# ouyangjiahong/representation-disentanglement

Measured on AMD Instinct MI355X. Metric: MR slices/sec (train step, recon+adv+latent losses), higher is better.
Workload: dtype f32

## Files before the change

representation-disentanglement_amd/csrc/mrdis_common.h:

```cpp
#pragma once
#include <hip/hip_runtime.h>
#include <stdint.h>
#include "../../include/mrdis.h"
#include "mrdis_device.h"
#include "mrdis_launchers.h"

#define MRDIS_CHECK_LAUNCH()                                     \
    do {                                                         \
        hipError_t e_ = hipGetLastError();                       \
        if (e_ != hipSuccess) return MRDIS_ELAUNCH;              \
    } while (0)

#define MRDIS_OPTIONS(X) \
    X(WINO, "wino", "MRDIS_WINO", 0, 1)  \
    X(NT_MB, "nt_mb", "MRDIS_NT_MB", 0, 128)  \
    X(WINO_PIPE, "wino_pipe", "MRDIS_WINO_PIPE", 0, 1)  \
    X(WINO_U, "wino_u", "MRDIS_WINO_U", 0, 1)  \
    X(WINO4, "wino4", "MRDIS_WINO4", 0, 1)  \
    X(WINO4R, "wino4r", "MRDIS_WINO4R", 0, 1)  \
    X(BCONV4, "bconv4", "MRDIS_BCONV4", 0, 1)  \
    X(SPLIT6, "split6", "MRDIS_SPLIT6", 0, 1)  \
    X(NO16, "debug_no16", "MRDIS_DEBUG_NO16", 1, 0) \
    X(NOTHIN, "debug_nothin", "MRDIS_DEBUG_NOTHIN", 1, 0) \
    X(NOC4, "debug_noc4", "MRDIS_DEBUG_NOC4", 1, 0) \
    X(NODMA, "debug_nodma", "MRDIS_DEBUG_NODMA", 1, 0) \
    X(NO16_3D, "debug_no16_3d", "MRDIS_DEBUG_NO16_3D", 1, 0) \
    X(BILGEN, "debug_bilgen", "MRDIS_DEBUG_BILGEN", 1, 0) \
    X(NOW16, "debug_now16", "MRDIS_DEBUG_NOW16", 1, 0) \
    X(NOPACK, "debug_nopack", "MRDIS_DEBUG_NOPACK", 1, 0)  \
    X(MODE, "debug_mode", "MRDIS_DEBUG_MODE", 0, -1) \
    X(BN, "debug_bn", "MRDIS_DEBUG_BN", 0, -1) \
    X(KC, "debug_kc", "MRDIS_DEBUG_KC", 0, -1) \
    X(BM, "debug_bm", "MRDIS_DEBUG_BM", 0, -1) \
    X(C4_TW, "debug_c4_tw", "MRDIS_DEBUG_C4_TW", 0, -1) \
    X(WGSPLIT, "debug_wgsplit", "MRDIS_DEBUG_WGSPLIT", 0, -1) \
    X(BN3, "debug_bn3", "MRDIS_DEBUG_BN3", 0, -1) \
    X(KC3, "debug_kc3", "MRDIS_DEBUG_KC3", 0, -1) \
    X(C4_GRID, "c4_grid", "MRDIS_C4_GRID", 0, 0)  \
    X(C4_BLOCKS, "debug_c4_blocks", "MRDIS_DEBUG_C4_BLOCKS", 0, -1)  \
    X(ZS_GRID, "zsearch_grid", "MRDIS_ZSEARCH_GRID", 0, 0)  \
    X(VOLGEN, "debug_volgen", "MRDIS_DEBUG_VOLGEN", 1, 0)
#define MRDIS_X_OPT_ID(id, name, env, is_flag, dflt) MRDIS_OPT_##id,
enum { MRDIS_OPTIONS(MRDIS_X_OPT_ID) MRDIS_OPT_COUNT };
long long mrdis_opt(int id);
void mrdis_opt_note(int id, long long value);

#define MRDIS_COUNTERS(X) \
    X(WINO, "wino") X(WINO_SPADE, "wino_spade") X(WINO2, "wino2") X(WINO2_SPADE, "wino2_spade") X(WINO4, "wino4") X(WINO4_SPADE, "wino4_spade") X(WINO4N, "wino4n") \
    X(WINO4R, "wino4r") X(WINO_WGRAD, "wino_wgrad") X(WINO_WGRAD2, "wino_wgrad2") X(WINO4_WGRAD, "wino4_wgrad") X(BCONV3, "bconv3") X(BCONV3_SPADE, "bconv3_spade") \
    X(BCONV4, "bconv4") X(BCONV4_SPADE, "bconv4_spade") X(SPLIT6_C4, "split6_c4") X(SPLIT6_C16, "split6_c16") X(SPLIT6_WGRAD16, "split6_wgrad16") X(SPLIT6_CO4, "split6_co4") \
    X(SPLIT6_C3D, "split6_c3d") X(SPLIT6_W3D, "split6_w3d") X(SPLIT6_TAP, "split6_tap") X(ZSEARCH, "zsearch") \
    X(CONV2SRC, "conv2src") X(ANA_ACT, "ana_act")  \
    X(KL, "kl") X(AVGPOOL, "avgpool")  \
    X(CHATT, "chatt") X(SYMDIFF, "symdiff") X(RGATE, "rgate")  \
    X(DIRECT3D, "direct3d") X(C3D16, "c3d16") X(WGRAD3D, "wgrad3d") X(WGRAD3D16, "wgrad3d16") X(WINO_WGRAD3D, "wino_wgrad3d")  \
    X(VOLGATHER, "volgather")  \
    X(FGCOUNT, "fgcount") X(PATCHORIGIN, "patchorigin") X(PATCHGATHER, "patchgather")  \
    X(PATCHWARP, "patchwarp")  \
    X(LOSS3D, "loss3d") X(SEGCOUNTS, "segcounts")  \
    X(SEGACCUM, "segaccum") X(SEGLABELS, "seglabels")  \
    X(TILEACCUM, "tileaccum") X(TILELABELS, "tilelabels")  \
    X(SYNTHACCUM, "synthaccum") X(SYNTHFINISH, "synthfinish")  \
    X(SEG2DLABELS, "seg2dlabels") X(SEG2DFINISH, "seg2dfinish")  \
    X(FUSE, "fuse")  \
    X(REGSURF, "regsurf") X(EDT, "edt") X(SURFHIST, "surfhist")  \
    X(CCLABEL, "cclabel") X(CCCLEAN, "ccclean")  \
// ... 39 lines not shown
```

representation-disentanglement_amd/csrc/mrdis_conv.hip:

```cpp
#include "mrdis_common.h"
#include "mrdis_tapconv.h"
#include "mrdis_s6conv.h"
#include "mrdis_wino4.h"
#include <stdlib.h>
#include <type_traits>

__device__ float g_mrdis_zero_page[64];
#define TC_TAB_INTS 320

template <int KC, int BN, int MODE, int BM, int SK = 1>
__device__ __forceinline__ void tapconv_body(const TapConvParams& p, const int bx, const int gx) {
    constexpr int S = KC + 1;
    constexpr int WAVES_N = (BN == 32) ? 1 : 2;
    constexpr int WAVES_M = 4 / WAVES_N;
    constexpr int MSUB = (BM / 32) / WAVES_M;
    constexpr int NSUB = (BN / 32) / WAVES_N;
    constexpr int KCW = KC / SK;
    static_assert(SK == 1 || (SK == 2 && BN == 32 && BM == 128 && MODE == 1 && KC >= 8), "split-K form: 64 positions x 32 couts, two waves per 32 x 32 block");
    extern __shared__ __attribute__((aligned(16))) float smem[];
    int* tab_in = reinterpret_cast<int*>(smem);
    int* tab_out = tab_in + BM;
    int* tap_xoff = tab_in + 2 * BM;
    int* tap_widx = tab_in + 2 * BM + 16;
    float* ws = smem + (2 * BM + 64);
// ... 2268 lines not shown
    WgradPlan pl;
    if (plan_wgrad(pl, N, H, W, Ci, Ci, Co, kh, kw, stride, pad)) return 0;
    size_t need = wgrad_need(pl);
    { const size_t nb = mrdis_bwgrad_workspace(N, H, W, Ci, Co, kh, kw, stride, pad); if (nb > need) need = nb; }
    if (kh == 3 && kw == 3 && stride == 1 && pad == 1) {
        const size_t nw = mrdis_wino_wgrad_workspace(N, H, W, Ci, Co);
        if (nw > need) need = nw;
        const size_t n16 = mrdis_wgrad16_workspace(N, H, W, Ci, Co);
        if (n16 > need) need = n16;
        const size_t n4 = mrdis_wgrad_c4_workspace(N, H, W, Ci, Co);
        if (n4 > need) need = n4;
        const size_t n4b = mrdis_wgrad_co4b_workspace(N, H, W, Ci, Co);
        if (n4b > need) need = n4b;
    }
    { const size_t n2 = mrdis_wgrad_s2_workspace(N, H, W, Ci, Co, kh, kw, stride, pad); if (n2 > need) need = n2; }
    if (kh == 1 && kw == 1 && stride == 1 && pad == 0) { const size_t n1 = mrdis_pw_wgrad_workspace((long long)N * H * W, Ci, Co, 1); if (n1 > need) need = n1; }
    return need;
}

template <int J>
static int launch_wgrad_t(const WgradPlan& pl, hipStream_t s) {
    if (pl.dma) {
        if (!mrdis_lds_optin((const void*)wgrad_dma_kernel<J>, 96 * 1024)) return MRDIS_ELAUNCH;
        const bool x_ok = (pl.p.ldx % 4 == 0) && (((uintptr_t)pl.p.x & 15) == 0);
        const bool dy_ok = (pl.p.lddy % 4 == 0) && (((uintptr_t)pl.p.dy & 15) == 0);
        if (x_ok && dy_ok) {
            MRDIS_LAUNCH((wgrad_dma_kernel<J>), dim3(pl.p.splits * pl.p.base), dim3(256), pl.lds_dma, s, pl.p, pl.XR);
            MRDIS_CHECK_LAUNCH();
            return MRDIS_OK;
        }
// ... 40 lines not shown
    if (kh == 3 && kw == 3 && stride == 1 && pad == 1 && Ci == 4) {
        rc = mrdis_run_wgrad_c4(x, ldx, dy, lddy, dw_tck, dbias, workspace, workspace_bytes, N, H, W, Ci, Co, accumulate_bias, 0, (hipStream_t)stream);
        if (rc != MRDIS_EUNSUPPORTED) return rc;
    }
    if (kh == 3 && kw == 3 && stride == 1 && pad == 1 && Co <= 16) {
        rc = mrdis_run_wgrad16(x, ldx, dy, lddy, dw_tck, dbias, workspace, workspace_bytes, N, H, W, Ci, Co, accumulate_bias, (hipStream_t)stream);
        if (rc != MRDIS_EUNSUPPORTED) return rc;
    }
    if (kh == 1 && kw == 1 && stride == 1 && pad == 0) {
        rc = mrdis_run_pw_wgrad(x, ldx, dy, lddy, dw_tck, dbias, workspace, workspace_bytes, (long long)N * H * W, Ci, Co, accumulate_bias, 0, (hipStream_t)stream);
        if (rc != MRDIS_EUNSUPPORTED) return rc;
    }
    if (stride == 2 && Ci <= 7) {
        rc = mrdis_run_wgrad_s2(x, ldx, dy, lddy, dw_tck, dbias, workspace, workspace_bytes, N, H, W, Ci, Co, kh, kw, stride, pad, accumulate_bias,
                                (hipStream_t)stream);
        if (rc != MRDIS_EUNSUPPORTED) return rc;
    }
    if (wino_wgrad_wanted(N, H, W, Ci, Co, kh, kw, stride, pad)) {
        rc = mrdis_run_wino_wgrad(x, ldx, dy, lddy, dw_tck, dbias, workspace, workspace_bytes, N, H, W, Ci, Co, accumulate_bias, (hipStream_t)stream);
        if (rc != MRDIS_EUNSUPPORTED) return rc;
    }
    hipStream_t s = (hipStream_t)stream;
    WgradParams& p = pl.p;
    p.x = x; p.dy = dy; p.ldx = ldx; p.lddy = lddy;
    p.slab = reinterpret_cast<float*>(workspace);
    float* part = p.slab + pl.slab_floats;
    p.bias_slab = dbias ? part + pl.part_floats : nullptr;
    p.vec_x = (Ci % 4 == 0) && (ldx % 4 == 0) && (((uintptr_t)x & 15) == 0) && (p.CW % 4 == 0);
    p.vec_dy = (Co % 4 == 0) && (lddy % 4 == 0) && (((uintptr_t)dy & 15) == 0);
    const bool x_al = (ldx % 4 == 0) && (((uintptr_t)x & 15) == 0), dy_al = (lddy % 4 == 0) && (((uintptr_t)dy & 15) == 0);
// ... 486 lines not shown
```

representation-disentanglement_amd/csrc/mrdis_launchers.h:

```cpp
#pragma once
#include <hip/hip_runtime.h>
#include <stddef.h>

int mrdis_run_wino(const float* x, int ldx, const float* w, const float* bias, float* y, int ldy,
                   int N, int H, int W, int Ci, int Co, int flip, int lrelu, hipStream_t s);
int mrdis_run_wino3d(const float* x, int ldx, const float* w, const float* bias, const float* res, int ldres, float* y, int ldy,
                     int N, int D, int H, int W, int Ci, int Co, int flip, hipStream_t s);
size_t mrdis_wino_wgrad_workspace(int N, int H, int W, int Ci, int Co);
int mrdis_run_wino_wgrad(const float* x, int ldx, const float* dy, int lddy, float* dw_tck, float* dbias, void* workspace,
                         size_t workspace_bytes, int N, int H, int W, int Ci, int Co, int accumulate_bias, hipStream_t s);
size_t mrdis_wino_wgrad3d_workspace(int N, int D, int H, int W, int Ci, int Co);
int mrdis_run_wino_wgrad3d(const float* x, int ldx, const float* dy, int lddy, float* dw_tck, float* dbias, void* workspace,
                           size_t workspace_bytes, int N, int D, int H, int W, int Ci, int Co, hipStream_t s);

int mrdis_run_wino2(const float* x, int ldx, const float* w, const float* bias, float* y, int ldy,
                    int N, int H, int W, int Ci, int Co, int flip, int lrelu, hipStream_t s, const float* u_img);
int mrdis_run_wino2_spade(const float* x, int ldx, const float* w, const float* bias, const float* z, int ldz, const float* mean, const float* rstd,
                          float* mix, int ldmix, float* gamma, int ldg, int N, int H, int W, int Ci, int C, hipStream_t s, const float* u_img);

int mrdis_run_wino4(const float* x, int ldx, const float* bias, float* y, int ldy, int N, int H, int W, int Ci, int Co, int lrelu,
                    hipStream_t s, const float* u_img);
int mrdis_run_wino4n(const float* x, int ldx, const float* bias, float* y, int ldy, int N, int H, int W, int Ci, int Co, int lrelu,
                     hipStream_t s, const float* u_img);
int mrdis_run_wino4_spade(const float* x, int ldx, const float* bias, const float* z, int ldz, const float* mean, const float* rstd,
                          float* mix, int ldmix, float* gamma, int ldg, int N, int H, int W, int Ci, int C, hipStream_t s, const float* u_img);
// ... 48 lines not shown
```

representation-disentanglement_amd/csrc/mrdis_wino.h:

```cpp
#pragma once
#include "mrdis_common.h"

struct WinoWgradParams {
    const float* x; const float* dy; float* slab; float* bias_slab;
    int N, H, W, Ci, ldx, Co, lddy;
    int nby, nbx, nblocks;
    int nCiB, nCoB, splits;
    int D, kd;
};

int mrdis_launch_wino_wgrad2(const WinoWgradParams& p, hipStream_t s);

int mrdis_launch_wino4_wgrad(WinoWgradParams& p, int max_splits, hipStream_t s);
```

representation-disentanglement_amd/csrc/mrdis_wino.hip:

```cpp
#include "mrdis_common.h"
#include "mrdis_wino.h"
#include <stdlib.h>

struct WinoParams {
    const float* in; const float* w; const float* bias; float* out;
    const float* res; int ldres;
    int D;
    int N, H, W, Cin, ldin, Cout, ldout;
    int flip, lrelu, nt_out;
    int TBH, TBW;
    int nby, nbx, coTiles;
};

template <int CG, int TG, bool D3 = false>
__global__ __launch_bounds__(64 * CG * TG, (CG * TG == 8) ? 1 : 2) void wino_conv_kernel(const WinoParams p) {
    constexpr int KC = 8, NT = 64 * CG * TG;
    constexpr int RWP = 24;
    constexpr int BN = 32 * CG, T = 16 * TG;
    constexpr int TS = T + 16, US = BN + 16;
    constexpr int XR = NT == 512 ? 2 : 3;
    constexpr int UR = (KC * BN) / NT;
    extern __shared__ __attribute__((aligned(16))) float smem[];
    float* U = smem;
    float* V = U + 16 * KC * US;
// ... 443 lines not shown
        __syncthreads();
        float s_ = 0.f;
#pragma unroll
        for (int z = 0; z < ZR; ++z) s_ += bsum[z];
        float* red = smem;
        red[tid] = (tid < TB * COB || ZR > 1) ? s_ : 0.f;
        __syncthreads();
        if (tid < COB) {
            float t = 0.f;
            for (int k = tid; k < NT; k += COB) t += red[k];
            p.bias_slab[(long long)split * p.Co + co0 + tid] = t;
        }
    }
}

__global__ void wino_sum_slabs_kernel(const float* __restrict__ slab, float* __restrict__ dw, long long n, int nslab,
                                      const float* __restrict__ bslab, float* __restrict__ dbias, int Co, int accumulate_bias) {
    __shared__ float red[16][65];
    const long long i = (long long)blockIdx.x * 64 + threadIdx.x;
    const int SL = blockDim.y, y = threadIdx.y;
    float s_ = 0.f;
    if (i < n) {
        const float* src = slab + i + (long long)y * n;
        const long long step = (long long)SL * n;
        int k = y;
        for (; k + 3 * SL < nslab; k += 4 * SL, src += 4 * step) { const float a = src[0], b = src[step], c = src[2 * step], d = src[3 * step]; s_ += a; s_ += b; s_ += c; s_ += d; }
        for (; k < nslab; k += SL, src += step) s_ += *src;
    } else if (dbias != nullptr && i < n + Co) {
        const int co = (int)(i - n);
        for (int k = y; k < nslab; k += SL) s_ += bslab[(long long)k * Co + co];
    }
    red[y][threadIdx.x] = s_;
    __syncthreads();
    if (y == 0) {
        float t = 0.f;
        for (int k = 0; k < SL; ++k) t += red[k][threadIdx.x];
        if (i < n) dw[i] = t;
        else if (dbias != nullptr && i < n + Co) { const int co = (int)(i - n); dbias[co] = accumulate_bias ? dbias[co] + t : t; }
    }
}

struct WinoWgradPlan { WinoWgradParams p; int wci, wco; size_t lds; bool ok; };

static void plan_wino_wgrad(WinoWgradPlan& pl, int N, int H, int W, int Ci, int Co) {
    pl.ok = false;
    int wci, wco;
    if (Ci % 64 == 0 && Co % 64 == 0) { wci = 4; wco = 2; }
    else if (Ci % 64 == 0 && Co % 32 == 0) { wci = 4; wco = 1; }
    else if (Ci % 32 == 0 && Co % 64 == 0) { wci = 2; wco = 2; }
    else return;
    WinoWgradParams& p = pl.p;
    p = WinoWgradParams{};
// ... 2 lines not shown
    const long long nb = (long long)N * p.nby * p.nbx;
    if (nb > 0x7fffffffLL) return;
    p.nblocks = (int)nb;
    const int CIB = 16 * wci, COB = 32 * wco;
    p.nCiB = Ci / CIB; p.nCoB = Co / COB;
    const int target = (wci * wco == 8) ? 256 : 512;
    int splits = target / (p.nCiB * p.nCoB);
    if (splits < 1) splits = 1;
    if (splits > p.nblocks) splits = p.nblocks;
    p.splits = splits;
    pl.wci = wci; pl.wco = wco;
    pl.lds = sizeof(float) * ((size_t)16 * 8 * (CIB + 16) + (size_t)16 * 8 * (COB + 16) + (size_t)60 * (CIB + 4));
    pl.ok = true;
}

size_t mrdis_wino_wgrad_workspace(int N, int H, int W, int Ci, int Co) {
    WinoWgradPlan pl;
    plan_wino_wgrad(pl, N, H, W, Ci, Co);
    if (!pl.ok) return 0;
    return sizeof(float) * ((size_t)pl.p.splits * 9 * Ci * Co + (size_t)pl.p.splits * Co) + 256;
}

int mrdis_run_wino_wgrad(const float* x, int ldx, const float* dy, int lddy, float* dw_tck, float* dbias, void* workspace,
                         size_t workspace_bytes, int N, int H, int W, int Ci, int Co, int accumulate_bias, hipStream_t s) {
    WinoWgradPlan pl;
    plan_wino_wgrad(pl, N, H, W, Ci, Co);
    if (!pl.ok || ldx % 4 != 0 || (((uintptr_t)x) & 15) != 0) return MRDIS_EUNSUPPORTED;
    if (workspace_bytes < mrdis_wino_wgrad_workspace(N, H, W, Ci, Co) - 256) return MRDIS_EUNSUPPORTED;
    WinoWgradParams& p = pl.p;
    p.x = x; p.dy = dy; p.ldx = ldx; p.lddy = lddy;
    p.slab = reinterpret_cast<float*>(workspace);
    p.bias_slab = dbias ? p.slab + (size_t)p.splits * 9 * Ci * Co : nullptr;
    int rc2 = MRDIS_EUNSUPPORTED;
    {
        const int rc4 = mrdis_launch_wino4_wgrad(p, p.splits, s);
        if (rc4 == MRDIS_OK) rc2 = MRDIS_OK;
        else if (rc4 != MRDIS_EUNSUPPORTED) return rc4;
    }
    const int nblk = p.splits * p.nCiB * p.nCoB;
    if (rc2 != MRDIS_OK && pl.wci == 4 && pl.wco == 2 && mrdis_opt(MRDIS_OPT_WINO_PIPE)) {
        rc2 = mrdis_launch_wino_wgrad2(p, s);
        if (rc2 != MRDIS_OK && rc2 != MRDIS_EUNSUPPORTED) return rc2;
    }
#define WW_LAUNCH(a, b_, nt, kb) { if (!mrdis_lds_optin((const void*)wino_wgrad_kernel<a, b_>, kb * 1024)) return MRDIS_ELAUNCH; \
                                   mrdis_count(MRDIS_CNT_WINO_WGRAD); MRDIS_LAUNCH((wino_wgrad_kernel<a, b_>), dim3(nblk), dim3(nt), pl.lds, s, p); }
    if (rc2 == MRDIS_OK) {}
    else if (pl.wci == 4 && pl.wco == 2) WW_LAUNCH(4, 2, 512, 120)
    else if (pl.wci == 4) WW_LAUNCH(4, 1, 256, 80)
    else WW_LAUNCH(2, 2, 256, 80)
#undef WW_LAUNCH
    MRDIS_CHECK_LAUNCH();
    const long long n = 9LL * Ci * Co;
    int SL = 1;
    while (SL < 16 && SL * 4 <= p.splits) SL <<= 1;
    MRDIS_LAUNCH(wino_sum_slabs_kernel, dim3(mrdis_cdiv(n + (dbias ? Co : 0), 64)), dim3(64, SL), 0, s, p.slab, dw_tck, n, p.splits,
                       p.bias_slab, dbias, Co, accumulate_bias);
    MRDIS_CHECK_LAUNCH();
    return MRDIS_OK;
}

size_t mrdis_wino_wgrad3d_workspace(int N, int D, int H, int W, int Ci, int Co) { return mrdis_wino_wgrad_workspace(N * D, H, W, Ci, Co); }

int mrdis_run_wino_wgrad3d(const float* x, int ldx, const float* dy, int lddy, float* dw_tck, float* dbias, void* workspace,
                           size_t workspace_bytes, int N, int D, int H, int W, int Ci, int Co, hipStream_t s) {
    WinoWgradPlan pl;
    plan_wino_wgrad(pl, N * D, H, W, Ci, Co);
    if (!pl.ok || ldx % 4 != 0 || (((uintptr_t)x) & 15) != 0) return MRDIS_EUNSUPPORTED;
    if (workspace_bytes + 256 < mrdis_wino_wgrad3d_workspace(N, D, H, W, Ci, Co)) return MRDIS_EUNSUPPORTED;
    WinoWgradParams& p = pl.p;
    p.x = x; p.dy = dy; p.ldx = ldx; p.lddy = lddy; p.D = D;
    p.slab = reinterpret_cast<float*>(workspace);
// ... 3 lines not shown
                             : (const void*)wino_wgrad_kernel<2, 2, true>, w42 ? 120 * 1024 : 80 * 1024)) return MRDIS_ELAUNCH;
    const int nblk = p.splits * p.nCiB * p.nCoB;
    const long long n = 9LL * Ci * Co;
    int SL = 1;
    while (SL < 16 && SL * 4 <= p.splits) SL <<= 1;
    for (int kd = 0; kd < 3; ++kd) {
        p.kd = kd;
        p.bias_slab = (dbias && kd == 1) ? bias_slab : nullptr;
        mrdis_count(MRDIS_CNT_WINO_WGRAD3D);
        if (w42) MRDIS_LAUNCH((wino_wgrad_kernel<4, 2, true>), dim3(nblk), dim3(512), pl.lds, s, p);
        else if (pl.wci == 4) MRDIS_LAUNCH((wino_wgrad_kernel<4, 1, true>), dim3(nblk), dim3(256), pl.lds, s, p);
        else MRDIS_LAUNCH((wino_wgrad_kernel<2, 2, true>), dim3(nblk), dim3(256), pl.lds, s, p);
        MRDIS_CHECK_LAUNCH();
        float* db = p.bias_slab ? dbias : nullptr;
        MRDIS_LAUNCH(wino_sum_slabs_kernel, dim3(mrdis_cdiv(n + (db ? Co : 0), 64)), dim3(64, SL), 0, s, p.slab, dw_tck + kd * n, n, p.splits,
                           p.bias_slab, db, Co, 0);
        MRDIS_CHECK_LAUNCH();
    }
    return MRDIS_OK;
}
```

representation-disentanglement_amd/csrc/mrdis_wino4w.hip:

```cpp
#include "mrdis_wino.h"

namespace {
constexpr int W_NT = 512;
constexpr int W_VPP = 256, W_VBUF = 18 * W_VPP;
constexpr int W_ZPP = 512, W_ZBUF = 18 * W_ZPP;
constexpr int W_PIX = 32, W_RAW = 128 * W_PIX;
constexpr int W_NXI = 4;
constexpr size_t W4W_LDS = sizeof(float) * (2 * W_VBUF + 2 * W_ZBUF + 3 * W_RAW);
template <int V_> struct WIC { static constexpr int value = V_; };
__device__ __forceinline__ f32x2 ww_ld2(const float* p) { return *(const volatile __attribute__((address_space(3))) f32x2*)p; }
__device__ __forceinline__ void ww_st2(float* p, f32x2 v) { *(volatile __attribute__((address_space(3))) f32x2*)p = v; }
constexpr unsigned WW_OOB = 0xfffffff0u;
}

struct Wino4WgradParams {
    const float* x; const float* dy; float* slab; float* bias_slab;
    int N, H, W, Ci, ldx, Co, lddy;
    int ngy, ngx, ngroups;
    int nCiB, nCoB, splits;
    int prio;
    int s_n, s_gy, s_gx;
    unsigned long long* dbg; int dbg_cap;
};

__global__ __launch_bounds__(512, 2) void wino4_wgrad_kernel(const Wino4WgradParams p) {
    extern __shared__ __attribute__((aligned(16))) float smem[];
    float* const Vb = smem;
    float* const Zb = smem + 2 * W_VBUF;
    float* const Rb = Zb + 2 * W_ZBUF;

    const int tid = threadIdx.x, lane = tid & 63, l16 = lane & 15, kq = lane >> 4;
    const int wave = __builtin_amdgcn_readfirstlane(tid >> 6);
    int b_ = mrdis_xcd_remap((int)blockIdx.x, (int)gridDim.x);
    const int cob = b_ % p.nCoB; b_ /= p.nCoB;
    const int cib = b_ % p.nCiB;
    const int split = b_ / p.nCiB;
    const int ci0 = 32 * cib, co0 = 64 * cob;
    const int wi = wave & 1, wo = wave >> 1;
    const int a_off = kq * 64 + ((2 * (16 * wi + l16) + 32 * kq) & 63);
// ... 4 lines not shown
    const int p0_ = (4 * ty) * 10 + 4 * tx;
    const int v_src0 = p0_ * W_PIX + 4 * ((vc >> 2) ^ (p0_ & 4)) + (vc & 3);
    const int v_src1 = p0_ * W_PIX + 4 * ((vc >> 2) ^ (p0_ & 4) ^ 4) + (vc & 3);
    const int v_dst = t_ * 64 + ((2 * vc + 32 * t_) & 63);
    const int zc = 16 * (wave & 3) + l16;
    const int z_dst = t_ * 128 + ((2 * zc + 32 * t_) & 127);

    struct Cur { int n, gy, gx; };
    auto advance = [&](Cur& c) {
        c.gx += p.s_gx; if (c.gx >= p.ngx) { c.gx -= p.ngx; ++c.gy; }
        c.gy += p.s_gy; if (c.gy >= p.ngy) { c.gy -= p.ngy; ++c.n; }
        c.n += p.s_n;
    };
    Cur xcur, dcur;
    { int t = split; xcur.gx = t % p.ngx; t /= p.ngx; xcur.gy = t % p.ngy; xcur.n = t / p.ngy; dcur = xcur; }
    const __amdgpu_buffer_rsrc_t rs_x = mrdis_buffer_rsrc(p.x, mrdis_nhwc_bytes(p.N, p.H, p.W, p.ldx, p.Ci, 4));
    const __amdgpu_buffer_rsrc_t rs_dy = mrdis_buffer_rsrc(p.dy, mrdis_nhwc_bytes(p.N, p.H, p.W, p.lddy, p.Co, 4));

    float sc[62];
#pragma unroll
    for (int k = 0; k < 62; ++k) sc[k] = 0.f;
#define WW_D(ii, j) sc[5 * ((j) & 1) + (ii)]
#define WW_R(a, j) sc[10 + 6 * (a) + (j)]
#define WW_VO(k) sc[28 + (k)]
#define WW_DY(S, e) sc[16 * (S) + (e)]
#define WW_T(i, j) sc[32 + 4 * (i) + (j)]
#define WW_ZO(k) sc[56 + (k)]
    float bsum = 0.f;
    if ((p.prio == 1 && wave >= 4) || (p.prio == 2 && wave < 4)) __builtin_amdgcn_s_setprio(1);

    unsigned x_rel[W_NXI]; int x_yx[W_NXI];
#pragma unroll
    for (int j = 0; j < W_NXI; ++j) {
        const int slot = 8 * ((wave & 3) + 4 * j) + (lane >> 3), q = (lane & 7) ^ (slot & 4), ry = slot / 10, rx = slot - ry * 10;
        x_yx[j] = slot < 100 ? ((ry << 8) | rx) : -1;
        x_rel[j] = 4u * (unsigned)((ry * p.W + rx) * p.ldx + ci0 + 4 * q);
    }
    const unsigned lds_raw = (unsigned)(size_t)(__attribute__((address_space(3))) void*)Rb;
    auto dma_x = [&](int buf, int j) {
        const int h = 8 * xcur.gy - 1 + (x_yx[j] >> 8), w_ = 8 * xcur.gx - 1 + (x_yx[j] & 255);
        const bool ok = x_yx[j] >= 0 && xcur.n < p.N && (unsigned)h < (unsigned)p.H && (unsigned)w_ < (unsigned)p.W;
        const unsigned gb = 4u * (unsigned)(((xcur.n * p.H + 8 * xcur.gy - 1) * p.W + 8 * xcur.gx - 1) * p.ldx);
        const unsigned vo = ok ? gb + x_rel[j] : WW_OOB;
        const unsigned m0v = __builtin_amdgcn_readfirstlane(lds_raw + 4u * (unsigned)(buf * W_RAW) + 1024u * (unsigned)((wave & 3) + 4 * j));
        mrdis_buffer_lds_dma16(m0v, vo, rs_x);
        if (j == W_NXI - 1) advance(xcur);
    };
    auto v_read = [&](const float* Rr, int j, auto RH_) {
#pragma unroll
        for (int ii = 0; ii < 5; ++ii) { const int d_ = (decltype(RH_)::value + ii) * 10 + j; WW_D(ii, j) = Rr[((d_ & 4) ? v_src1 : v_src0) + d_ * W_PIX]; }
    };
    auto v_col = [&](int j, auto RH_) {
        const float e0 = WW_D(0, j), e1 = WW_D(1, j), e2 = WW_D(2, j), e3 = WW_D(3, j), e4 = WW_D(4, j);
        if constexpr (decltype(RH_)::value == 0) {
            const float a = fmaf(-4.f, e2, e4), b = fmaf(-4.f, e1, e3);
            WW_R(0, j) = fmaf(4.f, e0, fmaf(-5.f, e2, e4)); WW_R(1, j) = a + b; WW_R(2, j) = a - b;
        } else {
// ... 170 lines not shown
        float t = bsum;
        t += __shfl_xor(t, 16, 64);
        t += __shfl_xor(t, 32, 64);
        if (lane < 16 && co0 + zc < p.Co) p.bias_slab[(long long)split * p.Co + co0 + zc] = t;
    }
}

#ifdef WINO4_ABLATIONS
static unsigned long long* g_w4w_dbg = nullptr; static int g_w4w_dbg_cap = 0;
extern "C" void mrdis_debug_wino4w_stamps(void* buf, int cap_per_wave) { g_w4w_dbg = (unsigned long long*)buf; g_w4w_dbg_cap = cap_per_wave; }
#endif
int mrdis_launch_wino4_wgrad(WinoWgradParams& base, int max_splits, hipStream_t s) {
    const int opt = (int)mrdis_opt(MRDIS_OPT_WINO4);
    if (!opt || base.D != 0) return MRDIS_EUNSUPPORTED;
    if (base.Ci % 32 != 0 || base.Co % 64 != 0 || base.ldx % 4 != 0 || (((uintptr_t)base.x) & 15) != 0) return MRDIS_EUNSUPPORTED;
    if ((long long)base.N * base.H * base.W * base.ldx >= 0x3fffffffLL || (long long)base.N * base.H * base.W * base.lddy >= 0x3fffffffLL) return MRDIS_EUNSUPPORTED;
    Wino4WgradParams p{};
    p.prio = mrdis_opt(MRDIS_OPT_MODE) == 1001 ? 1 : (mrdis_opt(MRDIS_OPT_MODE) == 1002 ? 2 : 0);
    p.x = base.x; p.dy = base.dy; p.slab = base.slab; p.bias_slab = base.bias_slab;
    p.N = base.N; p.H = base.H; p.W = base.W; p.Ci = base.Ci; p.ldx = base.ldx; p.Co = base.Co; p.lddy = base.lddy;
    p.ngy = mrdis_cdiv(p.H, 8); p.ngx = mrdis_cdiv(p.W, 8);
    const long long ng = (long long)p.N * p.ngy * p.ngx;
    if (ng > 0x7fffffffLL) return MRDIS_EUNSUPPORTED;
    p.ngroups = (int)ng;
    p.nCiB = p.Ci / 32; p.nCoB = p.Co / 64;
    int splits = 256 / (p.nCiB * p.nCoB);
    if (splits < 1) splits = 1;
    if (splits > max_splits) splits = max_splits;
    if (splits > p.ngroups) splits = p.ngroups;
    if (p.H % 8 != 0 || p.W % 8 != 0) return MRDIS_EUNSUPPORTED;
    if (opt < 2 && (p.ngroups / splits < 24 || splits * p.nCiB * p.nCoB < 192 || p.H < 8 || p.W < 8)) return MRDIS_EUNSUPPORTED;
    p.splits = splits;
    { int t = splits; p.s_gx = t % p.ngx; t /= p.ngx; p.s_gy = t % p.ngy; p.s_n = t / p.ngy; }
    if (!mrdis_lds_optin((const void*)wino4_wgrad_kernel, (int)W4W_LDS)) return MRDIS_EUNSUPPORTED;
#ifdef WINO4_ABLATIONS
    p.dbg = g_w4w_dbg; p.dbg_cap = g_w4w_dbg_cap;
#endif
    mrdis_count(MRDIS_CNT_WINO4_WGRAD);
    MRDIS_LAUNCH(wino4_wgrad_kernel, dim3(splits * p.nCiB * p.nCoB), dim3(W_NT), W4W_LDS, s, p);
    MRDIS_CHECK_LAUNCH();
    base.splits = splits;
    return MRDIS_OK;
}
```

representation-disentanglement_amd/hip.py:

```python
import collections
import ctypes
import os

import torch

_HERE = os.path.dirname(os.path.abspath(__file__))
LIB_PATH = os.path.join(_HERE, 'csrc', 'libmrdis_hip.so')


class MrdisLibraryError(RuntimeError):
    pass


class MrdisError(RuntimeError):
    pass


_lib = None
_c = ctypes
_P, _I, _L, _F, _Z = _c.c_void_p, _c.c_int, _c.c_longlong, _c.c_float, _c.c_size_t

_SIGS = {
    'mrdis_strerror': (_c.c_char_p, [_I]),
    'mrdis_version': (_I, []),
# ... 168 lines not shown
def options_snapshot():
    return {n: get_option(n) for n in OPTION_NAMES}


def options_restore(snap):
    for n, v in snap.items():
        if get_option(n) != v:
            set_option(n, v)


KERNEL_FAMILIES = WINO_FAMILIES = ('wino', 'wino_spade', 'wino2', 'wino2_spade', 'wino4', 'wino4_spade', 'wino4n', 'wino4r', 'wino_wgrad', 'wino_wgrad2', 'wino4_wgrad', 'bconv3', 'bconv3_spade', 'bconv4', 'bconv4_spade',
                                   'split6_c4', 'split6_c16', 'split6_wgrad16', 'split6_co4', 'split6_c3d', 'split6_w3d', 'split6_tap',
                                   'all',
                                   'zsearch')
VARIANT_FAMILIES = ('conv2src', 'ana_act')
LATENT_FAMILIES = ('kl', 'avgpool')
OUTDEC_FAMILIES = ('chatt', 'symdiff', 'rgate')
CONV3D_FAMILIES = ('direct3d', 'c3d16', 'wgrad3d', 'wgrad3d16', 'wino_wgrad3d')
DATA_FAMILIES = ('volgather',)
PATCH_FAMILIES = ('fgcount', 'patchorigin', 'patchgather')
PATCH_MAX_CLASSES = 8
WARP_FAMILIES = ('patchwarp',)
LOSS3D_FAMILIES = ('loss3d', 'segcounts')
SEGVOL_FAMILIES = ('segaccum', 'seglabels')
TILEPRED_FAMILIES = ('tileaccum', 'tilelabels')
TILE_FLIPS = 1 | 4 | 8
SYNTH_FAMILIES = ('synthaccum', 'synthfinish')
SEG2D_FAMILIES = ('seg2dlabels', 'seg2dfinish')
FUSE_FAMILIES = ('fuse',)
SURFDIST_FAMILIES = ('regsurf', 'edt', 'surfhist')
CC_FAMILIES = ('cclabel', 'ccclean')
LESION_FAMILIES = ('dilate', 'lesmatch', 'lesexpand')
PREP_FAMILIES = ('prepstats', 'prepwrite')
EXPORT_FAMILIES = ('export',)
ELEM_FAMILIES = ('stat_vec', 'stat_scalar', 'stat_interp', 'spade_up2_onepass', 'spade_up2_twopass', 'bil_fwd_x2', 'bil_fwd_general',
                 'bil_bwd_x2', 'bil_bwd_tight3', 'bil_bwd_tight5', 'bil_bwd_general', 'elem_v1')
LAUNCH_COUNTERS = (WINO_FAMILIES + VARIANT_FAMILIES + LATENT_FAMILIES + OUTDEC_FAMILIES + CONV3D_FAMILIES + DATA_FAMILIES + PATCH_FAMILIES + WARP_FAMILIES + LOSS3D_FAMILIES + SEGVOL_FAMILIES + TILEPRED_FAMILIES
                    + SYNTH_FAMILIES + SEG2D_FAMILIES + FUSE_FAMILIES + SURFDIST_FAMILIES + CC_FAMILIES + PREP_FAMILIES + EXPORT_FAMILIES + LESION_FAMILIES)
ALL_COUNTERS = LAUNCH_COUNTERS + ELEM_FAMILIES
SYNTH_MAX_SRC = 8
SEG2D_MAX_SETS = 16
SEG2D_MAX_VIEWS = 2
SEG2D_FLIPS = {'': 0, 'h': 1, 'w': 2}
FUSE_MAX_SRC = 8
FUSE_METHODS = ('mean', 'max', 'mean-max-min')
EDT_FAR = 1 << 30
EDT_MAX_SRC = 8
EDT_MAX_EXTENT = 1024
SURF_MAX_REGIONS = 4
CC_MAX_EXTENT = 1024
CC_LABEL_LAUNCHES = 3
CC_CONNECTIVITIES = (6, 18, 26)
# ... 1778 lines not shown
```

Baseline: 252.4.

## Route 4x4 stride-2 and narrow-Ci wgrad through Winograd via reindexing

```diff
diff --git a/representation-disentanglement_amd/csrc/mrdis_common.h b/representation-disentanglement_amd/csrc/mrdis_common.h
--- a/representation-disentanglement_amd/csrc/mrdis_common.h
+++ b/representation-disentanglement_amd/csrc/mrdis_common.h
@@ -28,7 +28,7 @@
     X(BILGEN, "debug_bilgen", "MRDIS_DEBUG_BILGEN", 1, 0) \
     X(NOW16, "debug_now16", "MRDIS_DEBUG_NOW16", 1, 0) \
     X(NOPACK, "debug_nopack", "MRDIS_DEBUG_NOPACK", 1, 0)  \
-    X(MODE, "debug_mode", "MRDIS_DEBUG_MODE", 0, -1) \
+    X(MODE, "debug_mode", "MRDIS_DEBUG_MODE", 0, -1)  \
     X(BN, "debug_bn", "MRDIS_DEBUG_BN", 0, -1) \
     X(KC, "debug_kc", "MRDIS_DEBUG_KC", 0, -1) \
     X(BM, "debug_bm", "MRDIS_DEBUG_BM", 0, -1) \
@@ -50,6 +50,7 @@
     X(WINO4R, "wino4r") X(WINO_WGRAD, "wino_wgrad") X(WINO_WGRAD2, "wino_wgrad2") X(WINO4_WGRAD, "wino4_wgrad") X(BCONV3, "bconv3") X(BCONV3_SPADE, "bconv3_spade") \
     X(BCONV4, "bconv4") X(BCONV4_SPADE, "bconv4_spade") X(SPLIT6_C4, "split6_c4") X(SPLIT6_C16, "split6_c16") X(SPLIT6_WGRAD16, "split6_wgrad16") X(SPLIT6_CO4, "split6_co4") \
     X(SPLIT6_C3D, "split6_c3d") X(SPLIT6_W3D, "split6_w3d") X(SPLIT6_TAP, "split6_tap") X(ZSEARCH, "zsearch") \
+    X(WGRAD_MIRROR, "wgrad_mirror") X(WGRAD_S2D, "wgrad_s2d")  \
     X(CONV2SRC, "conv2src") X(ANA_ACT, "ana_act")  \
     X(KL, "kl") X(AVGPOOL, "avgpool")  \
     X(CHATT, "chatt") X(SYMDIFF, "symdiff") X(RGATE, "rgate")  \
diff --git a/representation-disentanglement_amd/csrc/mrdis_conv.hip b/representation-disentanglement_amd/csrc/mrdis_conv.hip
--- a/representation-disentanglement_amd/csrc/mrdis_conv.hip
+++ b/representation-disentanglement_amd/csrc/mrdis_conv.hip
@@ -2306,6 +2306,10 @@
         if (n4b > need) need = n4b;
     }
     { const size_t n2 = mrdis_wgrad_s2_workspace(N, H, W, Ci, Co, kh, kw, stride, pad); if (n2 > need) need = n2; }
+    if (kh == 4 && kw == 4 && stride == 2 && pad == 1) {
+        const size_t nd = mrdis_wino_wgrad_s2d_workspace(N, H, W, Ci, Co);
+        if (nd > need) need = nd;
+    }
     if (kh == 1 && kw == 1 && stride == 1 && pad == 0) { const size_t n1 = mrdis_pw_wgrad_workspace((long long)N * H * W, Ci, Co, 1); if (n1 > need) need = n1; }
     return need;
 }
@@ -2376,6 +2380,10 @@
     if (stride == 2 && Ci <= 7) {
         rc = mrdis_run_wgrad_s2(x, ldx, dy, lddy, dw_tck, dbias, workspace, workspace_bytes, N, H, W, Ci, Co, kh, kw, stride, pad, accumulate_bias,
                                 (hipStream_t)stream);
+        if (rc != MRDIS_EUNSUPPORTED) return rc;
+    }
+    if (kh == 4 && kw == 4 && stride == 2 && pad == 1 && mrdis_opt(MRDIS_OPT_WINO) != 0) {
+        rc = mrdis_run_wino_wgrad_s2d(x, ldx, dy, lddy, dw_tck, dbias, workspace, workspace_bytes, N, H, W, Ci, Co, accumulate_bias, (hipStream_t)stream);
         if (rc != MRDIS_EUNSUPPORTED) return rc;
     }
     if (wino_wgrad_wanted(N, H, W, Ci, Co, kh, kw, stride, pad)) {
diff --git a/representation-disentanglement_amd/csrc/mrdis_launchers.h b/representation-disentanglement_amd/csrc/mrdis_launchers.h
--- a/representation-disentanglement_amd/csrc/mrdis_launchers.h
+++ b/representation-disentanglement_amd/csrc/mrdis_launchers.h
@@ -9,6 +9,9 @@
 size_t mrdis_wino_wgrad_workspace(int N, int H, int W, int Ci, int Co);
 int mrdis_run_wino_wgrad(const float* x, int ldx, const float* dy, int lddy, float* dw_tck, float* dbias, void* workspace,
                          size_t workspace_bytes, int N, int H, int W, int Ci, int Co, int accumulate_bias, hipStream_t s);
+size_t mrdis_wino_wgrad_s2d_workspace(int N, int H, int W, int C, int Co);
+int mrdis_run_wino_wgrad_s2d(const float* x, int ldx, const float* dy, int lddy, float* dw_tck, float* dbias, void* workspace,
+                             size_t workspace_bytes, int N, int H, int W, int C, int Co, int accumulate_bias, hipStream_t s);
 size_t mrdis_wino_wgrad3d_workspace(int N, int D, int H, int W, int Ci, int Co);
 int mrdis_run_wino_wgrad3d(const float* x, int ldx, const float* dy, int lddy, float* dw_tck, float* dbias, void* workspace,
                            size_t workspace_bytes, int N, int D, int H, int W, int Ci, int Co, hipStream_t s);
diff --git a/representation-disentanglement_amd/csrc/mrdis_wino.h b/representation-disentanglement_amd/csrc/mrdis_wino.h
--- a/representation-disentanglement_amd/csrc/mrdis_wino.h
+++ b/representation-disentanglement_amd/csrc/mrdis_wino.h
@@ -7,6 +7,7 @@
     int nby, nbx, nblocks;
     int nCiB, nCoB, splits;
     int D, kd;
+    int s2dC;
 };
 
 int mrdis_launch_wino_wgrad2(const WinoWgradParams& p, hipStream_t s);
diff --git a/representation-disentanglement_amd/csrc/mrdis_wino.hip b/representation-disentanglement_amd/csrc/mrdis_wino.hip
--- a/representation-disentanglement_amd/csrc/mrdis_wino.hip
+++ b/representation-disentanglement_amd/csrc/mrdis_wino.hip
@@ -481,28 +481,44 @@
     }
 }
 
+enum { WSUM_PLAIN = 0, WSUM_MIRROR = 1, WSUM_S2D = 2 };
 __global__ void wino_sum_slabs_kernel(const float* __restrict__ slab, float* __restrict__ dw, long long n, int nslab,
-                                      const float* __restrict__ bslab, float* __restrict__ dbias, int Co, int accumulate_bias) {
+                                      const float* __restrict__ bslab, float* __restrict__ dbias, int Co, int accumulate_bias,
+                                      int nbslab, int map, int Ci) {
     __shared__ float red[16][65];
     const long long i = (long long)blockIdx.x * 64 + threadIdx.x;
     const int SL = blockDim.y, y = threadIdx.y;
+    long long dst = i;
+    if (map == WSUM_MIRROR && i < n) {
+        const int ci = (int)(i % Ci); const long long r = i / Ci;
+        const int co = (int)(r % Co), t = (int)(r / Co);
+        dst = ((long long)(8 - t) * Ci + ci) * Co + co;
+    } else if (map == WSUM_S2D && i < n) {
+        const int co = (int)(i % Co); const long long r = i / Co;
+        const int cq = (int)(r % (4 * Ci)), t = (int)(r / (4 * Ci));
+        const int py = cq / (2 * Ci), px = (cq / Ci) & 1, c = cq % Ci;
+        const int a = 2 * (t / 3) - 1 + py, b = 2 * (t % 3) - 1 + px;
+        dst = ((unsigned)a < 4u && (unsigned)b < 4u) ? ((long long)(4 * a + b) * Ci + c) * Co + co : -1;
+    }
     float s_ = 0.f;
     if (i < n) {
-        const float* src = slab + i + (long long)y * n;
-        const long long step = (long long)SL * n;
-        int k = y;
-        for (; k + 3 * SL < nslab; k += 4 * SL, src += 4 * step) { const float a = src[0], b = src[step], c = src[2 * step], d = src[3 * step]; s_ += a; s_ += b; s_ += c; s_ += d; }
-        for (; k < nslab; k += SL, src += step) s_ += *src;
+        if (dst >= 0) {
+            const float* src = slab + i + (long long)y * n;
+            const long long step = (long long)SL * n;
+            int k = y;
+            for (; k + 3 * SL < nslab; k += 4 * SL, src += 4 * step) { const float a = src[0], b = src[step], c = src[2 * step], d = src[3 * step]; s_ += a; s_ += b; s_ += c; s_ += d; }
+            for (; k < nslab; k += SL, src += step) s_ += *src;
+        }
     } else if (dbias != nullptr && i < n + Co) {
         const int co = (int)(i - n);
-        for (int k = y; k < nslab; k += SL) s_ += bslab[(long long)k * Co + co];
+        for (int k = y; k < nbslab; k += SL) s_ += bslab[(long long)k * Co + co];
     }
     red[y][threadIdx.x] = s_;
     __syncthreads();
     if (y == 0) {
         float t = 0.f;
         for (int k = 0; k < SL; ++k) t += red[k][threadIdx.x];
-        if (i < n) dw[i] = t;
+        if (i < n) { if (dst >= 0) dw[dst] = t; }
         else if (dbias != nullptr && i < n + Co) { const int co = (int)(i - n); dbias[co] = accumulate_bias ? dbias[co] + t : t; }
     }
 }
@@ -535,11 +551,71 @@
     pl.ok = true;
 }
 
+constexpr int WCS_ROWS = 1024, WCS_NT = 256;
+__global__ __launch_bounds__(WCS_NT) void wino_dy_colsum_kernel(const float* __restrict__ dy, int lddy, long long npix, int Co, long long chunk, float* __restrict__ part) {
+    __shared__ float4 red[WCS_NT];
+    const int tid = threadIdx.x, Q = Co >> 2, L = WCS_NT / Q, q = tid % Q, l = tid / Q;
+    float4 s_ = make_float4(0.f, 0.f, 0.f, 0.f);
+    if (l < L) {
+        const long long p0 = (long long)blockIdx.x * chunk, p1 = p0 + chunk < npix ? p0 + chunk : npix;
+#pragma unroll 8
+        for (long long px = p0 + l; px < p1; px += L) {
+            const float4 v = *reinterpret_cast<const float4*>(dy + px * lddy + 4 * q);
+            s_.x += v.x; s_.y += v.y; s_.z += v.z; s_.w += v.w;
+        }
+    }
+    red[tid] = s_;
+    __syncthreads();
+    if (tid < Q) {
+        float4 t = red[tid];
+        for (int k = 1; k < L; ++k) { const float4 v = red[k * Q + tid]; t.x += v.x; t.y += v.y; t.z += v.z; t.w += v.w; }
+        *reinterpret_cast<float4*>(part + (long long)blockIdx.x * Co + 4 * tid) = t;
+    }
+}
+
 size_t mrdis_wino_wgrad_workspace(int N, int H, int W, int Ci, int Co) {
     WinoWgradPlan pl;
     plan_wino_wgrad(pl, N, H, W, Ci, Co);
     if (!pl.ok) return 0;
-    return sizeof(float) * ((size_t)pl.p.splits * 9 * Ci * Co + (size_t)pl.p.splits * Co) + 256;
+    const size_t colsum = (pl.wci == 4 && pl.wco == 1) ? (size_t)WCS_ROWS * Co : 0;
+    return sizeof(float) * ((size_t)pl.p.splits * 9 * Ci * Co + (size_t)pl.p.splits * Co + colsum) + 256;
+}
+
+static int wgrad_reindex_paths() {
+    const long long md = mrdis_opt(MRDIS_OPT_MODE);
+    return (md <= -4100 && md >= -4103) ? (int)(-4100 - md) : 3;
+}
+
+static int wino_sum_lanes(int splits) {
+    int SL = 1;
+    while (SL < 16 && SL * 4 <= splits) SL <<= 1;
+    return SL;
+}
+
+static int run_wino4_wgrad_mirror(const WinoWgradPlan& pl, float* dw_tck, float* dbias, int accumulate_bias, hipStream_t s) {
+    const WinoWgradParams& p = pl.p;
+    if (!(wgrad_reindex_paths() & 1) || p.lddy % 4 != 0 || (((uintptr_t)p.dy) & 15) != 0 || p.Co / 4 > WCS_NT) return MRDIS_EUNSUPPORTED;
+    WinoWgradParams m = p;
+    m.x = p.dy; m.ldx = p.lddy; m.Ci = p.Co;
+    m.dy = p.x; m.lddy = p.ldx; m.Co = p.Ci;
+    m.bias_slab = nullptr;
+    const int rc = mrdis_launch_wino4_wgrad(m, p.splits, s);
+    if (rc != MRDIS_OK) return rc;
+    mrdis_count(MRDIS_CNT_WGRAD_MIRROR);
+    float* part = p.slab + (size_t)p.splits * 9 * p.Ci * p.Co + (size_t)p.splits * p.Co;
+    int rows = 0;
+    if (dbias) {
+        const long long npix = (long long)p.N * p.H * p.W;
+        rows = mrdis_cdiv(npix, 256) < WCS_ROWS ? mrdis_cdiv(npix, 256) : WCS_ROWS;
+        const long long chunk = (npix + rows - 1) / rows;
+        MRDIS_LAUNCH(wino_dy_colsum_kernel, dim3(rows), dim3(WCS_NT), 0, s, p.dy, p.lddy, npix, p.Co, chunk, part);
+        MRDIS_CHECK_LAUNCH();
+    }
+    const long long n = 9LL * p.Ci * p.Co;
+    MRDIS_LAUNCH(wino_sum_slabs_kernel, dim3(mrdis_cdiv(n + (dbias ? p.Co : 0), 64)), dim3(64, wino_sum_lanes(m.splits)), 0, s, p.slab, dw_tck, n, m.splits,
+                       part, dbias, p.Co, accumulate_bias, rows, (int)WSUM_MIRROR, p.Ci);
+    MRDIS_CHECK_LAUNCH();
+    return MRDIS_OK;
 }
 
 int mrdis_run_wino_wgrad(const float* x, int ldx, const float* dy, int lddy, float* dw_tck, float* dbias, void* workspace,
@@ -553,6 +629,10 @@
     p.slab = reinterpret_cast<float*>(workspace);
     p.bias_slab = dbias ? p.slab + (size_t)p.splits * 9 * Ci * Co : nullptr;
     int rc2 = MRDIS_EUNSUPPORTED;
+    if (pl.wci == 4 && pl.wco == 1) {
+        const int rcm = run_wino4_wgrad_mirror(pl, dw_tck, dbias, accumulate_bias, s);
+        if (rcm != MRDIS_EUNSUPPORTED) return rcm;
+    }
     {
         const int rc4 = mrdis_launch_wino4_wgrad(p, p.splits, s);
         if (rc4 == MRDIS_OK) rc2 = MRDIS_OK;
@@ -572,10 +652,37 @@
 #undef WW_LAUNCH
     MRDIS_CHECK_LAUNCH();
     const long long n = 9LL * Ci * Co;
-    int SL = 1;
-    while (SL < 16 && SL * 4 <= p.splits) SL <<= 1;
-    MRDIS_LAUNCH(wino_sum_slabs_kernel, dim3(mrdis_cdiv(n + (dbias ? Co : 0), 64)), dim3(64, SL), 0, s, p.slab, dw_tck, n, p.splits,
-                       p.bias_slab, dbias, Co, accumulate_bias);
+    MRDIS_LAUNCH(wino_sum_slabs_kernel, dim3(mrdis_cdiv(n + (dbias ? Co : 0), 64)), dim3(64, wino_sum_lanes(p.splits)), 0, s, p.slab, dw_tck, n, p.splits,
+                       p.bias_slab, dbias, Co, accumulate_bias, p.splits, (int)WSUM_PLAIN, Ci);
+    MRDIS_CHECK_LAUNCH();
+    return MRDIS_OK;
+}
+
+static bool wino_wgrad_s2d_geometry(int H, int W, int C, int Co) {
+    return C % 16 == 0 && Co % 64 == 0 && H % 16 == 0 && W % 16 == 0;
+}
+size_t mrdis_wino_wgrad_s2d_workspace(int N, int H, int W, int C, int Co) {
+    return wino_wgrad_s2d_geometry(H, W, C, Co) ? mrdis_wino_wgrad_workspace(N, H / 2, W / 2, 4 * C, Co) : 0;
+}
+int mrdis_run_wino_wgrad_s2d(const float* x, int ldx, const float* dy, int lddy, float* dw_tck, float* dbias, void* workspace,
+                             size_t workspace_bytes, int N, int H, int W, int C, int Co, int accumulate_bias, hipStream_t s) {
+    if (!(wgrad_reindex_paths() & 2) || !wino_wgrad_s2d_geometry(H, W, C, Co)) return MRDIS_EUNSUPPORTED;
+    if (ldx % 4 != 0 || (((uintptr_t)x) & 15) != 0) return MRDIS_EUNSUPPORTED;
+    if (C % 32 != 0 && ldx != C) return MRDIS_EUNSUPPORTED;
+    WinoWgradPlan pl;
+    plan_wino_wgrad(pl, N, H / 2, W / 2, 4 * C, Co);
+    if (!pl.ok) return MRDIS_EUNSUPPORTED;
+    if (workspace_bytes + 256 < mrdis_wino_wgrad_s2d_workspace(N, H, W, C, Co)) return MRDIS_EUNSUPPORTED;
+    WinoWgradParams& p = pl.p;
+    p.x = x; p.dy = dy; p.ldx = ldx; p.lddy = lddy; p.s2dC = C;
+    p.slab = reinterpret_cast<float*>(workspace);
+    p.bias_slab = dbias ? p.slab + (size_t)p.splits * 9 * 4 * C * Co : nullptr;
+    const int rc = mrdis_launch_wino4_wgrad(p, p.splits, s);
+    if (rc != MRDIS_OK) return rc;
+    mrdis_count(MRDIS_CNT_WGRAD_S2D);
+    const long long n = 36LL * C * Co;
+    MRDIS_LAUNCH(wino_sum_slabs_kernel, dim3(mrdis_cdiv(n + (dbias ? Co : 0), 64)), dim3(64, wino_sum_lanes(p.splits)), 0, s, p.slab, dw_tck, n, p.splits,
+                       p.bias_slab, dbias, Co, accumulate_bias, p.splits, (int)WSUM_S2D, C);
     MRDIS_CHECK_LAUNCH();
     return MRDIS_OK;
 }
@@ -609,7 +716,7 @@
         MRDIS_CHECK_LAUNCH();
         float* db = p.bias_slab ? dbias : nullptr;
         MRDIS_LAUNCH(wino_sum_slabs_kernel, dim3(mrdis_cdiv(n + (db ? Co : 0), 64)), dim3(64, SL), 0, s, p.slab, dw_tck + kd * n, n, p.splits,
-                           p.bias_slab, db, Co, 0);
+                           p.bias_slab, db, Co, 0, p.splits, (int)WSUM_PLAIN, Ci);
         MRDIS_CHECK_LAUNCH();
     }
     return MRDIS_OK;
diff --git a/representation-disentanglement_amd/csrc/mrdis_wino4w.hip b/representation-disentanglement_amd/csrc/mrdis_wino4w.hip
--- a/representation-disentanglement_amd/csrc/mrdis_wino4w.hip
+++ b/representation-disentanglement_amd/csrc/mrdis_wino4w.hip
@@ -21,8 +21,10 @@
     int prio;
     int s_n, s_gy, s_gx;
     unsigned long long* dbg; int dbg_cap;
+    int x_row, x_pix, x_C, x_Wld;
 };
 
+template <bool S2D>
 __global__ __launch_bounds__(512, 2) void wino4_wgrad_kernel(const Wino4WgradParams p) {
     extern __shared__ __attribute__((aligned(16))) float smem[];
     float* const Vb = smem;
@@ -57,7 +59,7 @@
     };
     Cur xcur, dcur;
     { int t = split; xcur.gx = t % p.ngx; t /= p.ngx; xcur.gy = t % p.ngy; xcur.n = t / p.ngy; dcur = xcur; }
-    const __amdgpu_buffer_rsrc_t rs_x = mrdis_buffer_rsrc(p.x, mrdis_nhwc_bytes(p.N, p.H, p.W, p.ldx, p.Ci, 4));
+    const __amdgpu_buffer_rsrc_t rs_x = mrdis_buffer_rsrc(p.x, S2D ? mrdis_nhwc_bytes(p.N, 2 * p.H, 2 * p.W, p.ldx, p.x_C, 4) : mrdis_nhwc_bytes(p.N, p.H, p.W, p.ldx, p.Ci, 4));
     const __amdgpu_buffer_rsrc_t rs_dy = mrdis_buffer_rsrc(p.dy, mrdis_nhwc_bytes(p.N, p.H, p.W, p.lddy, p.Co, 4));
 
     float sc[62];
@@ -73,17 +75,21 @@
     if ((p.prio == 1 && wave >= 4) || (p.prio == 2 && wave < 4)) __builtin_amdgcn_s_setprio(1);
 
     unsigned x_rel[W_NXI]; int x_yx[W_NXI];
+    int x_c0 = ci0;
+    if constexpr (S2D) { const int c2 = ci0 % (2 * p.x_C); x_c0 = (ci0 / (2 * p.x_C)) * p.x_Wld + (c2 / p.x_C) * p.ldx + c2 % p.x_C; }
 #pragma unroll
     for (int j = 0; j < W_NXI; ++j) {
         const int slot = 8 * ((wave & 3) + 4 * j) + (lane >> 3), q = (lane & 7) ^ (slot & 4), ry = slot / 10, rx = slot - ry * 10;
         x_yx[j] = slot < 100 ? ((ry << 8) | rx) : -1;
-        x_rel[j] = 4u * (unsigned)((ry * p.W + rx) * p.ldx + ci0 + 4 * q);
+        if constexpr (S2D) x_rel[j] = 4u * (unsigned)(ry * p.x_row + rx * p.x_pix + x_c0 + 4 * q);
+        else x_rel[j] = 4u * (unsigned)((ry * p.W + rx) * p.ldx + ci0 + 4 * q);
     }
     const unsigned lds_raw = (unsigned)(size_t)(__attribute__((address_space(3))) void*)Rb;
     auto dma_x = [&](int buf, int j) {
         const int h = 8 * xcur.gy - 1 + (x_yx[j] >> 8), w_ = 8 * xcur.gx - 1 + (x_yx[j] & 255);
         const bool ok = x_yx[j] >= 0 && xcur.n < p.N && (unsigned)h < (unsigned)p.H && (unsigned)w_ < (unsigned)p.W;
-        const unsigned gb = 4u * (unsigned)(((xcur.n * p.H + 8 * xcur.gy - 1) * p.W + 8 * xcur.gx - 1) * p.ldx);
+        const unsigned gb = S2D ? 4u * (unsigned)((xcur.n * p.H + 8 * xcur.gy - 1) * p.x_row + (8 * xcur.gx - 1) * p.x_pix)
+                                : 4u * (unsigned)(((xcur.n * p.H + 8 * xcur.gy - 1) * p.W + 8 * xcur.gx - 1) * p.ldx);
         const unsigned vo = ok ? gb + x_rel[j] : WW_OOB;
         const unsigned m0v = __builtin_amdgcn_readfirstlane(lds_raw + 4u * (unsigned)(buf * W_RAW) + 1024u * (unsigned)((wave & 3) + 4 * j));
         mrdis_buffer_lds_dma16(m0v, vo, rs_x);
@@ -284,7 +290,9 @@
     const int opt = (int)mrdis_opt(MRDIS_OPT_WINO4);
     if (!opt || base.D != 0) return MRDIS_EUNSUPPORTED;
     if (base.Ci % 32 != 0 || base.Co % 64 != 0 || base.ldx % 4 != 0 || (((uintptr_t)base.x) & 15) != 0) return MRDIS_EUNSUPPORTED;
-    if ((long long)base.N * base.H * base.W * base.ldx >= 0x3fffffffLL || (long long)base.N * base.H * base.W * base.lddy >= 0x3fffffffLL) return MRDIS_EUNSUPPORTED;
+    const bool s2d = base.s2dC != 0;
+    if (s2d && (base.Ci != 4 * base.s2dC || base.s2dC % 16 != 0 || (base.s2dC % 32 != 0 && base.ldx != base.s2dC))) return MRDIS_EUNSUPPORTED;
+    if ((long long)base.N * base.H * base.W * base.ldx * (s2d ? 4 : 1) >= 0x3fffffffLL || (long long)base.N * base.H * base.W * base.lddy >= 0x3fffffffLL) return MRDIS_EUNSUPPORTED;
     Wino4WgradParams p{};
     p.prio = mrdis_opt(MRDIS_OPT_MODE) == 1001 ? 1 : (mrdis_opt(MRDIS_OPT_MODE) == 1002 ? 2 : 0);
     p.x = base.x; p.dy = base.dy; p.slab = base.slab; p.bias_slab = base.bias_slab;
@@ -302,12 +310,14 @@
     if (opt < 2 && (p.ngroups / splits < 24 || splits * p.nCiB * p.nCoB < 192 || p.H < 8 || p.W < 8)) return MRDIS_EUNSUPPORTED;
     p.splits = splits;
     { int t = splits; p.s_gx = t % p.ngx; t /= p.ngx; p.s_gy = t % p.ngy; p.s_n = t / p.ngy; }
-    if (!mrdis_lds_optin((const void*)wino4_wgrad_kernel, (int)W4W_LDS)) return MRDIS_EUNSUPPORTED;
+    if (s2d) { p.x_C = base.s2dC; p.x_Wld = 2 * p.W * p.ldx; p.x_row = 2 * p.x_Wld; p.x_pix = 2 * p.ldx; }
+    if (!mrdis_lds_optin(s2d ? (const void*)wino4_wgrad_kernel<true> : (const void*)wino4_wgrad_kernel<false>, (int)W4W_LDS)) return MRDIS_EUNSUPPORTED;
 #ifdef WINO4_ABLATIONS
     p.dbg = g_w4w_dbg; p.dbg_cap = g_w4w_dbg_cap;
 #endif
     mrdis_count(MRDIS_CNT_WINO4_WGRAD);
-    MRDIS_LAUNCH(wino4_wgrad_kernel, dim3(splits * p.nCiB * p.nCoB), dim3(W_NT), W4W_LDS, s, p);
+    if (s2d) MRDIS_LAUNCH(wino4_wgrad_kernel<true>, dim3(splits * p.nCiB * p.nCoB), dim3(W_NT), W4W_LDS, s, p);
+    else MRDIS_LAUNCH(wino4_wgrad_kernel<false>, dim3(splits * p.nCiB * p.nCoB), dim3(W_NT), W4W_LDS, s, p);
     MRDIS_CHECK_LAUNCH();
     base.splits = splits;
     return MRDIS_OK;
diff --git a/representation-disentanglement_amd/hip.py b/representation-disentanglement_amd/hip.py
--- a/representation-disentanglement_amd/hip.py
+++ b/representation-disentanglement_amd/hip.py
@@ -206,6 +206,7 @@
                                    'all',
                                    'zsearch')
 VARIANT_FAMILIES = ('conv2src', 'ana_act')
+REINDEX_FAMILIES = ('wgrad_mirror', 'wgrad_s2d')
 LATENT_FAMILIES = ('kl', 'avgpool')
 OUTDEC_FAMILIES = ('chatt', 'symdiff', 'rgate')
 CONV3D_FAMILIES = ('direct3d', 'c3d16', 'wgrad3d', 'wgrad3d16', 'wino_wgrad3d')
@@ -227,7 +228,7 @@
 EXPORT_FAMILIES = ('export',)
 ELEM_FAMILIES = ('stat_vec', 'stat_scalar', 'stat_interp', 'spade_up2_onepass', 'spade_up2_twopass', 'bil_fwd_x2', 'bil_fwd_general',
                  'bil_bwd_x2', 'bil_bwd_tight3', 'bil_bwd_tight5', 'bil_bwd_general', 'elem_v1')
-LAUNCH_COUNTERS = (WINO_FAMILIES + VARIANT_FAMILIES + LATENT_FAMILIES + OUTDEC_FAMILIES + CONV3D_FAMILIES + DATA_FAMILIES + PATCH_FAMILIES + WARP_FAMILIES + LOSS3D_FAMILIES + SEGVOL_FAMILIES + TILEPRED_FAMILIES
+LAUNCH_COUNTERS = (WINO_FAMILIES + REINDEX_FAMILIES + VARIANT_FAMILIES + LATENT_FAMILIES + OUTDEC_FAMILIES + CONV3D_FAMILIES + DATA_FAMILIES + PATCH_FAMILIES + WARP_FAMILIES + LOSS3D_FAMILIES + SEGVOL_FAMILIES + TILEPRED_FAMILIES
                     + SYNTH_FAMILIES + SEG2D_FAMILIES + FUSE_FAMILIES + SURFDIST_FAMILIES + CC_FAMILIES + PREP_FAMILIES + EXPORT_FAMILIES + LESION_FAMILIES)
 ALL_COUNTERS = LAUNCH_COUNTERS + ELEM_FAMILIES
 SYNTH_MAX_SRC = 8
```

Result: slower. 201.6 (-20.1%).
